# ivargr/kmer_mapper

Measured on AMD Instinct MI355X. Metric: M k-mers mapped/sec (whole node), k=31 150bp reads, higher is better.
Workload: dtype u64

## Files before the change

kmer_mapper_amd/csrc/kmm_radix.hpp:

```cpp
#pragma once
#include <type_traits>
#include "kmm_radix_plan.hpp"

constexpr int RX_NT = 512;
constexpr int RX_KPT = RX_B / RX_NT;
#ifndef RX_LPR2V
#define RX_LPR2V 16
#endif
constexpr int RX_LPR = RX_LPR2V;
constexpr int RX_NG = RX_NT / RX_LPR;
#ifndef RX_RB1
#define RX_RB1 4
#endif
#ifndef RX_RB2
#define RX_RB2 8
#endif
constexpr int RX_SUBCAP = 1024;
#ifndef RX_SUBCAP3V
#define RX_SUBCAP3V 3072
#endif
constexpr int RX_SUBCAP3 = RX_SUBCAP3V;
#ifndef RX_LPR3
#define RX_LPR3 16
#endif
// ... 775 lines not shown
    uint32_t jmax = n_items;
#pragma unroll
    for (int d = 32; d > 0; d >>= 1) {
        const uint32_t o = __shfl_xor(jmax, d);
        jmax = o > jmax ? o : jmax;
    }
    __syncthreads();
    if ((threadIdx.x & 63) == 0)
        s_wave8[threadIdx.x >> 6] = jmax;
    __syncthreads();
    if (c < F1) {
        rx.item_base[c] = ib;
        rx.work_base[c] = wb;
    }
    if (c == 0) {
        uint32_t m = s_wave8[0];
        for (int x = 1; x < 8; ++x)
            m = s_wave8[x] > m ? s_wave8[x] : m;
        rx.item_base[F1] = tot_items;
        rx.work_base[F1] = tot_rows;
        rx.ctrl[0] = tot_items;
        rx.ctrl[1] = tot_rows;
        rx.ctrl[2] = m;
    }
}

template <bool WITH_P>
__global__ void __launch_bounds__(256) k_rx_colscan(RxView rx)
{
    constexpr int RB = 32;
    constexpr int TB = WITH_P ? 32 : 64, CW = 256;
    static_assert(RX_CH % TB == 0 && TB % RB == 0, "a chunk is whole tiles, a tile whole register rounds");
    __shared__ uint32_t tP[WITH_P ? CW : 1][TB + 1];
    __shared__ uint16_t tS[CW][TB + 2];
    const uint32_t F1 = rx.F1, NB = rx.NB;
    const uint32_t b0 = blockIdx.x * RX_CH;
    const uint32_t b1 = b0 + RX_CH < NB ? b0 + RX_CH : NB;
    const size_t ld = F1 + 1;
    const uint32_t lane = threadIdx.x & 63, wave = threadIdx.x >> 6;
    {
    const uint32_t cb = blockIdx.y * CW;
    const uint32_t c = cb + threadIdx.x;
    const uint32_t nc = F1 - cb < (uint32_t)CW ? F1 - cb : (uint32_t)CW;
    uint32_t run = c < F1 ? rx.csum[(size_t)blockIdx.x * F1 + c] : 0u;
    const uint32_t ib = c < F1 ? rx.item_base[c] : 0u;
    for (uint32_t t0 = b0; t0 < b1; t0 += TB) {
        const uint32_t nb = b1 - t0 < (uint32_t)TB ? b1 - t0 : (uint32_t)TB;
        if (c < F1) {
#pragma unroll 1
            for (uint32_t r0 = 0; r0 < (uint32_t)TB; r0 += RB) {
                const uint16_t *p = rx.start1 + (size_t)(t0 + r0) * ld + c;
                uint32_t lo[RB], hi[RB];
#pragma unroll
                for (int u = 0; u < RB; ++u) {
                    lo[u] = r0 + (uint32_t)u < nb ? p[u * ld] : 0u;
                    hi[u] = r0 + (uint32_t)u < nb ? p[u * ld + 1] : 0u;
                }
#pragma unroll
                for (int u = 0; u < RB; ++u) {
                    const uint32_t cnt = hi[u] - lo[u];
                    if constexpr (WITH_P)
                        tP[threadIdx.x][r0 + u] = run;
                    tS[threadIdx.x][r0 + u] = (uint16_t)lo[u];
                    if (cnt) {
                        uint32_t m = (run + RX_B - 1) / RX_B;
                        while ((uint64_t)m * RX_B < (uint64_t)run + cnt) {
                            rx.item_desc[ib + m] = make_uint2(t0 + r0 + u, WITH_P ? c : run);
                            ++m;
                        }
                    }
                    run += cnt;
                }
            }
        }
        __syncthreads();
        if constexpr (WITH_P) {
            const uint32_t bi = lane & 31;
            for (uint32_t cc = wave * 2 + (lane >> 5); cc < nc; cc += 8) {
                if (bi < nb) {
                    rx.P1T[(size_t)(cb + cc) * (NB + 1) + t0 + bi] = tP[cc][bi];
                    rx.S1T[(size_t)(cb + cc) * NB + t0 + bi] = tS[cc][bi];
                }
            }
        } else {
            for (uint32_t cc = wave; cc < nc; cc += 4) {
                if (lane < nb)
                    rx.S1T[(size_t)(cb + cc) * NB + t0 + lane] = tS[cc][lane];
            }
        }
        __syncthreads();
    }
    }
}

constexpr int RX_TR2 = 32;
__global__ void __launch_bounds__(256) k_rx_tr2(RxView rx)
{
    __shared__ uint16_t tile[RX_TR2][RX_MAXF + 2];
    const uint32_t n_items = rx.ctrl[0], cols = rx.F2 + 1;
    const uint32_t i0 = blockIdx.x * RX_TR2;
    if (i0 >= n_items)
        return;
    const uint32_t ni = n_items - i0 < (uint32_t)RX_TR2 ? n_items - i0 : (uint32_t)RX_TR2;
    for (uint32_t e = threadIdx.x; e < ni * cols; e += 256)
        tile[e / cols][e % cols] = rx.start2[(size_t)i0 * cols + e];
    __syncthreads();
    const uint32_t it = threadIdx.x % RX_TR2, c0 = threadIdx.x / RX_TR2;
    if (it < ni)
        for (uint32_t col = c0; col < cols; col += 256 / RX_TR2)
            rx.start2T[(size_t)col * rx.max_items + i0 + it] = tile[it][col];
}

__global__ void __launch_bounds__(RX_NT, 4) k_rx_p2(IndexView iv, RxView rx)
{
    __shared__ uint64_t sbuf[RX_B];
    __shared__ uint32_t sub_src[RX_SUBCAP];
    __shared__ uint32_t sub_meta[RX_SUBCAP], s_wave8[2][RX_NT / 64];
    __shared__ __attribute__((aligned(8))) uint32_t s_cnt[RX_MAXF + 2 + 64];
    __shared__ uint32_t s_base[RX_MAXF + 1], s_wave[4];
    __shared__ uint32_t s_idx;
    const int tid = threadIdx.x, grp = tid / RX_LPR, lg = tid % RX_LPR;
    const uint32_t NB = rx.NB;
    uint32_t gathered = 0;
    uint32_t scan_flip = 0;
    const uint32_t spare = rx_spare_key();
    const int F2 = (int)rx.F2;
    const uint32_t cs = (rx.F1 + 7u) / 8u, limit = rx.ctrl[2] * cs;
    const uint32_t home = rx_xcc_id();
    if (tid <= F2)
        s_cnt[tid] = 0;
    if (tid == 0)
        s_cnt[RX_NT] = 0;
    struct Item {
        uint32_t valid, c, item, b0, lo, hi;
    };
    struct RunDesc {
        uint32_t vs, ve, st;
    };
    auto describe = [&](uint32_t sub, uint32_t idx) {
        Item d;
        d.valid = 0; d.c = 0; d.item = 0; d.b0 = 0; d.lo = 0; d.hi = 0;
        if (idx >= limit)
            return d;
        const uint32_t cj = idx / cs, cc = sub * cs + idx % cs;
        if (cc >= rx.F1)
            return d;
        const uint32_t ib = rx.item_base[cc];
        if (cj >= rx.item_base[cc + 1] - ib)
            return d;
        d.valid = 1;
        d.c = cc;
        d.item = ib + cj;
        d.b0 = rx.item_desc[d.item].x;
        d.lo = cj * RX_B;
        const uint32_t Tc = rx.T1[cc];
        d.hi = Tc - d.lo < (uint32_t)RX_B ? Tc : d.lo + RX_B;
        return d;
    };
    auto run_desc = [&](const Item &d, uint32_t bb) {
        RunDesc r;
        r.vs = 0xFFFFFFFFu; r.ve = 0xFFFFFFFFu; r.st = 0;
        const uint32_t b = bb + tid;
        if (d.valid && b < NB) {
            const uint32_t *P = rx.P1T + (size_t)d.c * (NB + 1);
            r.vs = P[b];
            r.ve = P[b + 1];
            r.st = rx.S1T[(size_t)d.c * NB + b];
        }
        return r;
    };
    RX_PT_DECL;
    for (uint32_t turn = 0; turn < 8u; ++turn) {
    const uint32_t sub = (home + turn) & 7u;
    uint32_t nxt = limit;
    if (tid == 0)
        nxt = rx_pop(rx.queue, sub, limit);
    if (tid == 0)
        s_idx = nxt;
    __syncthreads();
    uint32_t idx = s_idx;
    __syncthreads();
    if (idx >= limit)
        continue;
    if (tid == 0)
        nxt = rx_pop(rx.queue, sub, limit);
    Item it = describe(sub, idx);
    RunDesc rd = run_desc(it, it.b0);
    for (;;) {
        RX_PT(0);
        const uint32_t lo = it.lo, hi = it.hi, n = hi - lo;
        if (it.valid) {
            for (uint32_t bb = it.b0;; bb += RX_NT) {
                if (bb != it.b0)
                    rd = run_desc(it, bb);
                const uint32_t b = bb + tid;
                const uint32_t vs = rd.vs < hi ? rd.vs : hi;
                const bool live = vs < hi;
                const uint32_t ve = live ? rd.ve : vs;
                const uint32_t st = live ? rd.st : 0u;
                const uint32_t from = vs > lo ? vs : lo, to = ve < hi ? ve : hi;
                const uint32_t len = live && to > from ? to - from : 0u;
                const uint64_t src = (uint64_t)b * RX_B + st + (from - vs);
                uint32_t n_sub;
                const uint32_t last_more = (tid == RX_NT - 1 && live && ve < hi) ? 0x80000000u : 0u;
                const uint32_t pre = rx_scan_threads(rx_n_pieces<RX_LPR, true>(len, src) | last_more, s_wave8, scan_flip, &n_sub);
                const bool more = n_sub >> 31;
                n_sub &= 0x7FFFFFFFu;
                RX_PT(1);
                for (uint32_t win = 0; win < n_sub; win += RX_SUBCAP) {
                    rx_list_subruns<RX_LPR, true>(pre, len, src, from - lo, win, sub_src, sub_meta);
                    const uint32_t nw = n_sub - win < (uint32_t)RX_SUBCAP ? n_sub - win : (uint32_t)RX_SUBCAP;
                    rx_pad_list<RX_NG * RX_U2>(nw, sub_src, sub_meta);
                    __syncthreads();
                    for (uint32_t j0 = grp; j0 < nw; j0 += RX_NG * RX_U2) {
                        uint64_t x[RX_U2];
                        uint32_t meta[RX_U2], so[RX_U2];
#pragma unroll
                        for (int u = 0; u < RX_U2; ++u) {
                            meta[u] = sub_meta[j0 + u * RX_NG];
                            so[u] = sub_src[j0 + u * RX_NG];
                        }
#pragma unroll
                        for (int u = 0; u < RX_U2; ++u) {
                            const uint32_t rel = (uint32_t)lg - ((meta[u] >> 6) & 63u);
                            x[u] = rel < (meta[u] & 63u) ? RX_LOAD2(rx.buf1 + ((size_t)so[u] + lg)) : 0ull;
                        }
#pragma unroll
                        for (int u = 0; u < RX_U2; ++u) {
                            const uint32_t rel = (uint32_t)lg - ((meta[u] >> 6) & 63u);
                            if (rel < (meta[u] & 63u))
                                sbuf[(meta[u] >> 12) + rel] = x[u];
                        }
                    }
                    if (more || win + RX_SUBCAP < n_sub)
                        __syncthreads();
                }
                if (!more)
                    break;
            }
        }
        if (tid == 0)
            s_idx = nxt;
        __syncthreads();
        const uint32_t idx_n = s_idx;
        if (tid == 0 && idx_n < limit)
            nxt = rx_pop(rx.queue, sub, limit);
        const Item it_n = describe(sub, idx_n);
        RunDesc rd_n;
        rd_n.vs = 0xFFFFFFFFu; rd_n.ve = 0xFFFFFFFFu; rd_n.st = 0;
        if (it.valid) {
            uint64_t q[RX_KPT];
            uint32_t valid = 0;
#pragma unroll
            for (int i = 0; i < RX_KPT; ++i) {
                const uint32_t e = i * RX_NT + tid;
                q[i] = 0;
                if (e < n) {
                    q[i] = sbuf[e];
                    valid |= 1u << i;
                }
            }
            gathered += (uint32_t)__popc(valid);
            RX_PT(5);
            auto fine = [&](int i) {
                return ((valid >> i) & 1u) ? ((uint32_t)(q[i] >> rx.w) & (uint32_t)(F2 - 1)) : spare;
            };
            auto mid = [&]() { rd_n = run_desc(it_n, it_n.b0); };
            rx_sort_emit<RX_RB2, false, false>(q, fine, F2, sbuf, s_cnt, s_base, s_wave, rx.buf2 + (size_t)it.item * RX_B,
                            rx.start2 + (size_t)it.item * (F2 + 1) RX_PT_ARG2, mid);
        } else {
            rd_n = run_desc(it_n, it_n.b0);
            __syncthreads();
        }
        if (idx_n >= limit)
            break;
        idx = idx_n;
        it = it_n;
        rd = rd_n;
    }
    }
#ifndef RX_PT_P1
    RX_PT_END(iv, 10);
#endif
    rx_stat_add(iv, 2, gathered);
}

__device__ __forceinline__ uint32_t rx_fold2(uint32_t x)
{
    x = (x | (x >> 1)) & 0x55555555u;
    x = (x | (x >> 1)) & 0x33333333u;
    x = (x | (x >> 2)) & 0x0F0F0F0Fu;
    x = (x | (x >> 4)) & 0x00FF00FFu;
    return (x | (x >> 8)) & 0x0000FFFFu;
}
__device__ __forceinline__ uint32_t rx_fold4(uint32_t x)
{
    x = (x | (x >> 1) | (x >> 2) | (x >> 3)) & 0x11111111u;
    x = (x | (x >> 3)) & 0x03030303u;
    x = (x | (x >> 6)) & 0x000F000Fu;
    return (x | (x >> 12)) & 0xFFu;
}

constexpr int P2F_NT = 1024;
constexpr int P2F_KPT = RX_B / P2F_NT;

enum { P2F_NONE = 0, P2F_BITMAP = 1, P2F_SLOT = 2 };
template <int FILTER, bool FSMALL>
__global__ void __launch_bounds__(P2F_NT) k_rx_p2f(IndexView iv, RxView rx)
{
    constexpr bool SLOT = FILTER == P2F_SLOT;
    constexpr int CAPMAX = SLOT ? P2F_SLOTS : RX_B;
    __shared__ __attribute__((aligned(16))) uint32_t s_bits[SLOT ? P2F_SLOT_WORDS : (1 << P2F_LOGBITS) / 32];
    __shared__ __attribute__((aligned(16))) uint64_t sbuf[CAPMAX];
    __shared__ uint32_t t_vs[P2F_NT + 64];
    __shared__ uint32_t t_off[P2F_NT];
    __shared__ uint16_t t_aux[RX_B / 64 + 1];
    __shared__ uint32_t t_last;
    __shared__ uint32_t t_sbits[2][RX_B / 32];
    __shared__ uint32_t t_empty[2];
    __shared__ __attribute__((aligned(8))) uint32_t s_cnt2[2][RX_MAXF + 2 + 64];
    __shared__ uint32_t s_base[RX_MAXF + 1], s_wave[4];
    __shared__ uint32_t s_b0[P2F_KMAX], s_v0[P2F_KMAX];
    __shared__ uint32_t s_tot[3][P2F_NT / 64];
    __shared__ uint32_t s_idx;
    const int tid = threadIdx.x, lane = tid & 63;
    const uint32_t wave = (uint32_t)__builtin_amdgcn_readfirstlane(tid >> 6);
    const uint32_t NB = rx.NB;
    const int F2 = (int)rx.F2, w = rx.w;
    const uint32_t bmask = SLOT ? (1u << P2F_LOGBITS) - 1u : (1u << (rx.w + rx.f2)) - 1u;
    const uint32_t gs = (uint32_t)rx.occ_shift;
    constexpr bool nofilt = FILTER == P2F_NONE;
    const uint32_t nwords = nofilt ? 0u : SLOT ? (uint32_t)P2F_SLOT_WORDS
                                               : (((uint32_t)F2 << w) >> gs) / 32u;
    unsigned long long *const multi_stat =
        &iv.stats[(size_t)(blockIdx.x % KMM_STAT_SHARDS) * KMM_STAT_STRIDE + KMM_STAT_RX_MULTI];
    const uint32_t spare = rx_spare_key();
    uint32_t gathered = 0, dropped = 0;
    const uint32_t cs = (rx.F1 + 7u) / 8u;
    const uint32_t P2F_K = rx.p2f_k;
    const uint32_t limit = ((rx.ctrl[2] + P2F_K - 1u) / P2F_K) * cs;
    const uint32_t home = rx_xcc_id();
    if (tid <= F2)
        s_cnt2[0][tid] = s_cnt2[1][tid] = 0;
    RX_PT_DECL;

    struct RunDesc {
        uint32_t a, b;
    };
    for (uint32_t turn = 0; turn < 8u; ++turn) {
    const uint32_t sub = (home + turn) & 7u;
    for (;;) {
        if (tid == 0)
            s_idx = rx_pop(rx.queue, sub, limit);
        __syncthreads();
        const uint32_t idx = s_idx;
        __syncthreads();
        if (idx >= limit)
            break;
        const uint32_t cu = idx / cs, cc = sub * cs + idx % cs;
        if (cc >= rx.F1)
            continue;
        const uint32_t ib = rx.item_base[cc], n_items_c = rx.item_base[cc + 1] - ib;
        if (cu * P2F_K >= n_items_c)
            continue;
        const uint32_t j0 = cu * P2F_K;
        const uint32_t n_it = n_items_c - j0 < P2F_K ? n_items_c - j0 : P2F_K;
        const uint32_t Tc = rx.T1[cc];
        const uint16_t *S = rx.S1T + (size_t)cc * NB;
        const bool last_c = cc + 1u >= rx.F1;
        const uint16_t *SN = last_c ? rx.start1 + rx.F1 : S + NB;
        const uint32_t sn = last_c ? rx.F1 + 1u : 1u;
        if ((uint32_t)tid < n_it) {
            const uint2 d = rx.item_desc[ib + j0 + tid];
            s_b0[tid] = d.x;
            s_v0[tid] = d.y;
        }
        if (nofilt) {
        } else if (SLOT || gs == 0) {
            const uint4 *src = reinterpret_cast<const uint4 *>((SLOT ? rx.slots : rx.occ) + (size_t)cc * nwords);
            uint4 *dst = reinterpret_cast<uint4 *>(s_bits);
            for (uint32_t i = tid; i < nwords / 4u; i += P2F_NT)
                dst[i] = src[i];
            for (uint32_t i = (nwords & ~3u) + tid; !SLOT && i < nwords; i += P2F_NT)
                s_bits[i] = rx.occ[(size_t)cc * nwords + i];
        } else {
            const uint32_t *src = rx.occ + (((size_t)cc * nwords) << gs);
            for (uint32_t i = tid; i < nwords; i += P2F_NT) {
                uint32_t o = 0;
                if (gs == 1) {
                    const uint2 v = *reinterpret_cast<const uint2 *>(src + 2 * (size_t)i);
                    o = rx_fold2(v.x) | (rx_fold2(v.y) << 16);
                } else {
                    const uint4 v = *reinterpret_cast<const uint4 *>(src + 4 * (size_t)i);
                    o = rx_fold4(v.x) | (rx_fold4(v.y) << 8) | (rx_fold4(v.z) << 16) | (rx_fold4(v.w) << 24);
                }
                s_bits[i] = o;
            }
        }
        if (tid < 2 * (RX_B / 32))
            (&t_sbits[0][0])[tid] = 0u;
        if (tid < 2)
            t_empty[tid] = 0u;
        __syncthreads();

        auto item_lo = [&](uint32_t j) { return (j0 + j) * (uint32_t)RX_B; };
        auto item_n = [&](uint32_t j) {
            const uint32_t lo = (j0 + j) * (uint32_t)RX_B;
            return Tc - lo < (uint32_t)RX_B ? Tc - lo : (uint32_t)RX_B;
        };
        auto load_desc = [&](uint32_t bb) {
            RunDesc r;
            const uint32_t b = bb + tid;
            r.a = 0; r.b = 0;
            if (b < NB) {
                r.a = S[b];
                r.b = SN[b * sn];
            }
            return r;
        };
        auto prescan = [&](RunDesc &r, uint32_t row) {
            const uint32_t len = r.b - r.a;
            r.a |= len << 16;
            r.b = wave_scan_incl(len);
            if (lane == 63)
                s_tot[row][wave] = r.b;
        };
        auto put_table = [&](const RunDesc &r, uint32_t v0, uint32_t row, uint32_t lo, uint32_t hi, int mb = -1) {
            const uint32_t len = r.a >> 16, st = r.a & 0xFFFFu;
            const uint32_t tot = s_tot[row][lane & 15];
            const uint32_t below = (uint32_t)__builtin_amdgcn_readlane((int)wave_scan_incl((uint32_t)lane < wave ? tot : 0u), 15);
            const uint32_t vs = v0 + below + r.b - len, ve = vs + len;
            if (mb >= 0 && vs > lo && vs < hi) {
                if (len > 0u)
                    atomicOr(&t_sbits[mb][(vs - lo) >> 5], 1u << ((vs - lo) & 31u));
                else
                    t_empty[mb] = 1u;
            }
            t_vs[tid] = vs;
            t_off[tid] = (uint32_t)tid * RX_B + st - vs;
            if (tid == P2F_NT - 1) {
                t_vs[P2F_NT] = ve;
                if (ve < hi)
                    t_last = P2F_NT - 1;
            }
            const uint32_t from = vs > lo ? vs : lo, to = ve < hi ? ve : hi;
            if (from < to) {
                for (uint32_t a = (from - lo + 63u) >> 6; lo + (a << 6) < to; ++a)
                    t_aux[a] = (uint16_t)tid;
                if (to == hi)
                    t_last = (uint32_t)tid;
            }
        };
        auto fill = [&](auto merge_tag, uint32_t bb, uint32_t lo, uint32_t n, uint32_t c_lo, uint32_t c_hi,
                        uint64_t (&x)[P2F_KPT], int mb = -1) {
            constexpr bool MERGE = decltype(merge_tag)::value;
            const uint32_t c_end = lo + n < c_hi ? lo + n : c_hi;
            const uint32_t a0 = wave * 8u;
            uint32_t av = 0;
            {
                const uint32_t pa = lo + ((a0 + (uint32_t)lane) << 6);
                const uint32_t ia = a0 + ((uint32_t)lane <= 8u ? (uint32_t)lane : 8u);
                const uint32_t aux = t_aux[ia];
                av = pa < c_lo ? 0u : (pa < c_end ? aux : t_last);
            }
            uint32_t A[P2F_KPT + 1];
#pragma unroll
            for (int i = 0; i <= P2F_KPT; ++i)
                A[i] = (uint32_t)__builtin_amdgcn_readlane((int)av, i);
            uint32_t v[P2F_KPT], pos[P2F_KPT], len_max = 0;
            const uint32_t e0 = (a0 << 6) + (uint32_t)lane;
            auto n_below = [&](uint32_t bound) {
                const int32_t c = ((int32_t)(bound - lo) - (int32_t)e0 + 63) >> 6;
                return (uint32_t)(c < 0 ? 0 : (c > P2F_KPT ? P2F_KPT : c));
            };
            const uint32_t vmask = ((1u << n_below(c_end)) - 1u) & ~((1u << n_below(c_lo)) - 1u);
#pragma unroll
            for (int u = 0; u < P2F_KPT; ++u) {
                v[u] = lo + e0 + ((uint32_t)u << 6);
                pos[u] = A[u];
                const uint32_t len = A[u + 1] > A[u] ? A[u + 1] - A[u] : 0u;
                len_max = len > len_max ? len : len_max;
            }
            bool by_bits = false;
            if (!MERGE && mb >= 0 && t_empty[mb] == 0u) {
                by_bits = true;
                const uint32_t mw = t_sbits[mb][a0 * 2u + ((uint32_t)lane & 15u)];
#pragma unroll
                for (int u = 0; u < P2F_KPT; ++u) {
                    const uint32_t mlo = (uint32_t)__builtin_amdgcn_readlane((int)mw, 2 * u);
                    const uint32_t mhi = (uint32_t)__builtin_amdgcn_readlane((int)mw, 2 * u + 1);
                    const uint64_t m1 = (((uint64_t)mhi << 32) | mlo) >> 1;
                    pos[u] += __builtin_amdgcn_mbcnt_hi((uint32_t)(m1 >> 32), __builtin_amdgcn_mbcnt_lo((uint32_t)m1, 0u));
                }
                len_max = 0;
            }
            if (!by_bits) {
            const uint32_t span = A[P2F_KPT] > A[0] ? A[P2F_KPT] - A[0] : 0u;
            if (span < 64u) {
                const uint32_t sv = t_vs[A[0] + (uint32_t)lane];
#pragma unroll
                for (int u = 0; u < P2F_KPT; ++u) {
                    for (uint32_t i = A[u] + 1u; i <= A[u + 1]; ++i) {
                        const uint32_t st = (uint32_t)__builtin_amdgcn_readlane((int)sv, (int)(i - A[0]));
                        pos[u] += v[u] >= st ? 1u : 0u;
                    }
                }
                len_max = 0;
            }
            }
            for (uint32_t stp = len_max ? 1u << (31 - __builtin_clz(len_max)) : 0u; stp >= 1u; stp >>= 1) {
#pragma unroll
                for (int u = 0; u < P2F_KPT; ++u) {
                    const uint32_t cand = pos[u] + stp;
                    const uint32_t t = t_vs[cand <= A[u + 1] ? cand : A[u + 1]];
                    pos[u] = (cand <= A[u + 1] && t <= v[u]) ? cand : pos[u];
                }
            }
            const uint32_t bbs = (uint32_t)__builtin_amdgcn_readfirstlane((int)bb);
            const char *base = reinterpret_cast<const char *>(rx.buf1 + (size_t)bbs * RX_B);
            const size_t left = (size_t)NB * RX_B - (size_t)bbs * RX_B;
            const uint32_t lim = left > 0x1FFFFFFFull ? 0x1FFFFFFFu : (uint32_t)left - 1u;
#pragma unroll
            for (int u = 0; u < P2F_KPT; ++u) {
                uint32_t el = t_off[pos[u]] + v[u];
                el = el < lim ? el : lim;
                const uint64_t y = RX_LOAD2(reinterpret_cast<const uint64_t *>(base + (el << 3)));
                x[u] = (!MERGE || ((vmask >> u) & 1u)) ? y : x[u];
#if RX_PROBE_P2R
                if (u % RX_PROBE_P2R == 0) {
                    const size_t all = (size_t)NB * RX_B, far = ((size_t)bbs * RX_B + el + all / 2) % all;
                    const uint64_t z = RX_LOAD2(rx.buf1 + far);
                    asm volatile("" ::"v"(z));
                }
#endif
            }
            return vmask;
        };

        uint32_t cover = 0, b0 = 0;
        RunDesc rd;
        rd.a = 0; rd.b = 0;
        auto more_rounds = [&](uint32_t j, uint64_t (&x)[P2F_KPT], uint32_t &vm) {
            const uint32_t lo = item_lo(j), n = item_n(j), hi = lo + n;
            uint32_t bb = b0 + P2F_NT;
            while (cover < hi && bb < NB) {
                RunDesc r2 = load_desc(bb);
                prescan(r2, 2u);
                __syncthreads();
                put_table(r2, cover, 2u, lo, hi);
                __syncthreads();
                const uint32_t cover2 = t_vs[P2F_NT];
                vm |= fill(std::true_type(), bb, lo, n, cover, cover2, x);
                cover = cover2;
                bb += P2F_NT;
            }
            __syncthreads();
        };
        auto process = [&](uint32_t j, uint64_t (&xa)[P2F_KPT], uint32_t vma, uint64_t (&xb)[P2F_KPT], uint32_t &vmb) {
            const uint32_t item = ib + j0 + j;
            RX_PT(0);
            uint32_t keys[P2F_KPT], n_ok = 0;
            if (nofilt) {
#pragma unroll
                for (int u = 0; u < P2F_KPT; ++u) {
                    const uint32_t ok = (vma >> u) & 1u;
                    n_ok += ok;
                    keys[u] = ok ? __builtin_amdgcn_ubfe((uint32_t)xa[u], (uint32_t)w, (uint32_t)rx.f2) : spare;
                }
            } else {
#pragma unroll
                for (int u = 0; u < P2F_KPT; ++u) {
                    const uint32_t xl = (uint32_t)xa[u];
                    const uint32_t bit = SLOT ? rx_filter_slot(xl & bmask, xa[u] >> P2F_LOGBITS)
                                              : (xl & bmask) >> gs;
                    const uint32_t ok = (s_bits[bit >> 5] >> (bit & 31u)) & (vma >> u) & 1u;
                    n_ok += ok;
                    keys[u] = ok ? __builtin_amdgcn_ubfe(xl, (uint32_t)w, (uint32_t)rx.f2) : spare;
                }
            }
            gathered += (uint32_t)__popc(vma);
            dropped += (uint32_t)__popc(vma) - n_ok;
            RX_PT(5);
            if (j + 2u < n_it)
                prescan(rd, j & 1u);
            if (j + 1u < n_it) {
                const uint32_t lo1 = item_lo(j + 1u), n1 = item_n(j + 1u);
                b0 = s_b0[j + 1u];
                cover = t_vs[P2F_NT];
                vmb = fill(std::false_type(), b0, lo1, n1, lo1, cover, xb, (int)((j + 1u) & 1u));
                if (cover < lo1 + n1)
                    more_rounds(j + 1u, xb, vmb);
            }
            RX_PT(1);
            auto fine = [&](int i) { return keys[i]; };
            auto mid = [&]() {
                if (j + 2u < n_it) {
                    put_table(rd, s_v0[j + 2u], j & 1u, item_lo(j + 2u), item_lo(j + 2u) + item_n(j + 2u), (int)(j & 1u));
                    if (j + 3u < n_it)
                        rd = load_desc(s_b0[j + 3u]);
                }
            };
            rx_sort_emit<P2F_KPT, false, true, P2F_NT, false, decltype(fine), decltype(mid), (FSMALL ? 2 : 1), false, RxNoHook, CAPMAX>(
                xa, fine, F2, sbuf, s_cnt2[j & 1u], s_base, s_wave, rx.buf2 + (size_t)item * RX_B,
                rx.start2 + (size_t)item * (F2 + 1) RX_PT_ARG2, mid, P2F_KPT, -1, RxNoHook(),
                RX_PROBE_P2W ? rx.probe + (size_t)item * RX_B : nullptr, RX_PROBE_P2W, SLOT ? rx.p2f_cap : (uint32_t)RX_B,
                SLOT ? multi_stat : nullptr);
            if (tid < RX_B / 32)
                t_sbits[(j + 1u) & 1u][tid] = 0u;
            if (tid == 0)
                t_empty[(j + 1u) & 1u] = 0u;
        };

        uint64_t x0[P2F_KPT], x1[P2F_KPT];
        uint32_t vm0 = 0, vm1 = 0;
        b0 = s_b0[0];
        rd = load_desc(b0);
        prescan(rd, 0u);
        __syncthreads();
        put_table(rd, s_v0[0], 0u, item_lo(0), item_lo(0) + item_n(0), 0);
        if (n_it > 1u) {
            rd = load_desc(s_b0[1]);
            prescan(rd, 1u);
        }
        __syncthreads();
        cover = t_vs[P2F_NT];
        vm0 = fill(std::false_type(), b0, item_lo(0), item_n(0), item_lo(0), cover, x0, 0);
        __syncthreads();
        if (cover < item_lo(0) + item_n(0))
            more_rounds(0, x0, vm0);
        if (tid < RX_B / 32)
            t_sbits[0][tid] = 0u;
        if (tid == 0)
            t_empty[0] = 0u;
        if (n_it > 1u) {
            put_table(rd, s_v0[1], 1u, item_lo(1), item_lo(1) + item_n(1), 1);
            if (n_it > 2u)
                rd = load_desc(s_b0[2]);
        }
        __syncthreads();
        for (uint32_t j = 0; j < n_it; j += 2u) {
            process(j, x0, vm0, x1, vm1);
            if (j + 1u < n_it)
                process(j + 1u, x1, vm1, x0, vm0);
        }
    }
    }
#ifndef RX_PT_P1
    RX_PT_END(iv, 10);
#endif
    rx_stat_add(iv, 2, gathered);
    rx_stat_add(iv, KMM_STAT_RX_DROPPED, dropped);
}

#ifdef RX_P3_FP_STATS
#define RX_P3_KEY_READ(cond) key_reads += (cond) ? 1u : 0u
#else
#define RX_P3_KEY_READ(cond)
#endif
template <int WMAX, int ECAP, int WPS, typename DirT, int SUBCAP = RX_SUBCAP3, bool P16 = false, bool FP = false>
__global__ void __launch_bounds__(RX_NT, WPS) k_rx_p3(IndexView iv, RxView rx, int max_freq)
{
    static_assert(!P16 || sizeof(DirT) == 2, "the 16-bit directory is copied as it is");
    __shared__ uint32_t sfp[FP ? (ECAP + 8) / 4 : 1];
    __shared__ __attribute__((aligned(4))) DirT sdir[WMAX + 2];
    __shared__ uint64_t skeys[ECAP];
    __shared__ uint32_t scnt[ECAP];
    __shared__ uint32_t sub_list[SUBCAP];
    __shared__ uint32_t s_wb[RX_MAXF + 1], s_wave8[2][RX_NT / 64];
    __shared__ uint32_t s_idx;
    const int tid = threadIdx.x, grp = tid / RX_LPR_P3, lg = tid % RX_LPR_P3;
    const uint32_t n_rows = rx.ctrl[1], F1 = rx.F1, F2 = rx.F2;
    const uint32_t W = 1u << rx.w;
    const uint64_t M = iv.modulo;
    for (uint32_t i = tid; i <= F1; i += RX_NT)
        s_wb[i] = rx.work_base[i];
    const uint32_t gs = (F2 + 7u) / 8u, limit = n_rows * gs;
    unsigned long long *counters = rx.queue + 128;
    const uint32_t home = rx_xcc_id();
    uint32_t hits = 0, probed = 0, scan_flip = 0;
#ifdef RX_P3_FP_STATS
    uint32_t key_reads = 0;
#endif
    const int sh = rx.w + rx.f2;
    __syncthreads();
    struct Slice {
        uint32_t valid, g, e0, ne, it0, n_it, over, tot, fmax;
        uint64_t h0;
    };
    auto describe = [&](uint32_t sub, uint32_t idx) {
        Slice d;
        d.valid = 0; d.g = 0; d.e0 = 0; d.ne = 0; d.it0 = 0; d.n_it = 0; d.h0 = 0; d.over = 0; d.tot = 0; d.fmax = 0xFFFFu;
        if (idx >= limit)
            return d;
        const uint32_t row = idx / gs, g = sub * gs + idx % gs;
        uint32_t c_lo = 0, c_hi = F1;
        while (c_hi - c_lo > 1) {
            const uint32_t mid = (c_lo + c_hi) >> 1;
            if (s_wb[mid] <= row)
                c_lo = mid;
            else
                c_hi = mid;
        }
        const uint32_t c = c_lo;
        const uint32_t f2c = rx.PF - c * F2 < F2 ? rx.PF - c * F2 : F2;
        if (g >= f2c)
            return d;
        const uint32_t chunk = row - s_wb[c];
        d.valid = 1;
        d.g = g;
        d.h0 = (uint64_t)(c * F2 + g) << rx.w;
        uint32_t e1;
        if (P16) {
            d.e0 = rx.slice_e0[c * F2 + g];
            e1 = rx.slice_e0[c * F2 + g + 1u];
            d.fmax = rx.slice_fmax ? (uint32_t)rx.slice_fmax[c * F2 + g] : 0xFFFFu;
        } else {
            d.e0 = rx.pstart[d.h0];
            e1 = rx.pstart[d.h0 + W < M ? d.h0 + W : M];
        }
        d.tot = e1 - d.e0;
        d.ne = e1 - d.e0 < (uint32_t)ECAP ? e1 - d.e0 : (uint32_t)ECAP;
        d.over = e1 - d.e0 > (uint32_t)ECAP ? 1u : 0u;
        d.it0 = rx.item_base[c] + chunk * RX_IC;
        const uint32_t it_end = rx.item_base[c + 1];
        d.n_it = it_end - d.it0 < (uint32_t)RX_IC ? it_end - d.it0 : (uint32_t)RX_IC;
        return d;
    };
    RX_PT_DECL;
    for (uint32_t turn = 0; turn < 8u; ++turn) {
    const uint32_t sub = (home + turn) & 7u;
    uint32_t nxt = limit;
    if (tid == 0)
        nxt = rx_pop(counters, sub, limit);
    if (tid == 0)
        s_idx = nxt;
    __syncthreads();
    const uint32_t idx_first = s_idx;
    __syncthreads();
    if (idx_first >= limit)
        continue;
    if (tid == 0)
        nxt = rx_pop(counters, sub, limit);
    Slice sl = describe(sub, idx_first);
    for (;;) {
        RX_PT(0);
        const uint32_t g = sl.g, e0 = sl.e0, ne = sl.ne, it0 = sl.it0, n_it = sl.n_it;
        const uint64_t h0 = sl.h0;
        uint32_t rf[RX_IC / RX_NT], rt[RX_IC / RX_NT];
#pragma unroll
        for (int j = 0; j < RX_IC / RX_NT; ++j)
            rf[j] = rt[j] = 0;
        if (sl.valid) {
        uint32_t dv[WMAX / RX_NT + 1];
        uint64_t kv[ECAP / RX_NT];
        uint32_t fv[ECAP / RX_NT];
#ifndef RX_P3_FMAX
#define RX_P3_FMAX 1
#endif
        const bool need_f = RX_P3_FMAX == 0 || (int)sl.fmax > max_freq;
        if (P16) {
            const uint32_t *p32 = reinterpret_cast<const uint32_t *>(rx.pstart16 + h0);
#pragma unroll
            for (int j = 0; j < WMAX / 2 / RX_NT; ++j) {
                const uint32_t i = tid + j * RX_NT;
                dv[j] = i < W / 2u ? p32[i] : 0u;
            }
            if (W < 2u)
                dv[0] = tid == 0 ? (uint32_t)rx.pstart16[h0] : 0u;
        } else {
#pragma unroll
            for (int j = 0; j <= WMAX / RX_NT; ++j) {
                const uint32_t i = tid + j * RX_NT;
                dv[j] = i <= W ? rx.pstart[h0 + i < M ? h0 + i : M] : 0u;
            }
        }
#pragma unroll
        for (int j = 0; j < ECAP / RX_NT; ++j) {
            const uint32_t i = tid + j * RX_NT;
            kv[j] = i < ne ? rx.pkeys[(size_t)e0 + i] : 0ull;
            fv[j] = i < ne && need_f ? rx.pfreq[(size_t)e0 + i] : 0u;
        }
        const uint16_t *rfp = rx.start2T + (size_t)g * rx.max_items + it0;
        const uint16_t *rtp = rfp + rx.max_items;
#pragma unroll
        for (int j = 0; j < RX_IC / RX_NT; ++j) {
            const uint32_t i = tid + j * RX_NT;
            rf[j] = i < n_it ? rfp[i] : 0u;
            rt[j] = i < n_it ? rtp[i] : 0u;
        }
        if (P16) {
            uint32_t *sd32 = reinterpret_cast<uint32_t *>(sdir);
#pragma unroll
            for (int j = 0; j < WMAX / 2 / RX_NT; ++j) {
                const uint32_t i = tid + j * RX_NT;
                if (i < W / 2u)
                    sd32[i] = dv[j];
            }
            if (W < 2u && tid == 0)
                sdir[0] = (DirT)dv[0];
            if (tid == 0)
                sdir[W] = (DirT)sl.tot;
        } else {
#pragma unroll
            for (int j = 0; j <= WMAX / RX_NT; ++j) {
                const uint32_t i = tid + j * RX_NT;
                if (i <= W)
                    sdir[i] = (DirT)(dv[j] - e0);
            }
        }
#pragma unroll
        for (int j = 0; j < ECAP / RX_NT; ++j) {
            const uint32_t i = tid + j * RX_NT;
            if (i < ne) {
                skeys[i] = kv[j];
                if constexpr (FP)
                    reinterpret_cast<uint8_t *>(sfp)[i] = (uint8_t)rx_p3_fp(kv[j] >> sh);
                scnt[i] = (int)fv[j] <= max_freq ? 0u : RX_FILTERED;
            }
        }
        }
        RX_PT(1);
        if (tid == 0)
            s_idx = nxt;
        __syncthreads();
        const uint32_t idx_n = s_idx;
        if (tid == 0 && idx_n < limit)
            nxt = rx_pop(counters, sub, limit);
        const Slice sl_n = describe(sub, idx_n);
        auto probe_bucket_hbm = [&](uint64_t q, uint32_t st, uint32_t cn) {
            for (uint32_t j = 0; j < cn; ++j) {
                const size_t e = (size_t)e0 + st + j;
                if (rx.pkeys[e] == q && (int)rx.pfreq[e] <= max_freq) {
                    atomicAdd(&rx.ecnt[e], 1u);
                    ++hits;
                }
            }
        };
        if (sl.valid) {
        {
            constexpr int NR = RX_IC / RX_NT;
            uint32_t len[NR], np[NR], np_sum = 0, src[NR];
#pragma unroll
            for (int j = 0; j < NR; ++j) {
                len[j] = rt[j] - rf[j];
                src[j] = (uint32_t)(tid + j * RX_NT) * (uint32_t)RX_B + rf[j];
                np[j] = (len[j] + (uint32_t)RX_LPR_P3 - 1u) / (uint32_t)RX_LPR_P3;
                np_sum += np[j];
            }
            const char *wbase = reinterpret_cast<const char *>(rx.buf2 + (size_t)__builtin_amdgcn_readfirstlane((int)it0) * RX_B);
            uint32_t n_sub;
            const uint32_t pre = rx_scan_threads(np_sum, s_wave8, scan_flip, &n_sub);
            for (uint32_t win = 0; win < n_sub; win += SUBCAP) {
                uint32_t first = pre;
#pragma unroll
                for (int j = 0; j < NR; ++j) {
                    const uint32_t j0 = first > win ? first : win;
                    const uint32_t j1 = first + np[j] < win + (uint32_t)SUBCAP ? first + np[j] : win + (uint32_t)SUBCAP;
                    for (uint32_t q = j0; q < j1; ++q) {
                        const uint32_t done = (q - first) * (uint32_t)RX_LPR_P3;
                        const uint32_t n = len[j] - done < (uint32_t)RX_LPR_P3 ? len[j] - done : (uint32_t)RX_LPR_P3;
                        sub_list[q - win] = ((src[j] + done) << 5) | n;
                    }
                    first += np[j];
                }
                const uint32_t nw = n_sub - win < (uint32_t)SUBCAP ? n_sub - win : (uint32_t)SUBCAP;
                constexpr uint32_t STEP = RX_NG3 * RX_U;
                static_assert(SUBCAP % STEP == 0, "a padded list must fit the window");
                const uint32_t n_bat = (nw + STEP - 1u) / STEP;
                for (uint32_t i = nw + tid; i < n_bat * STEP; i += RX_NT)
                    sub_list[i] = 0u;
                __syncthreads();
                RX_PT(2);
                auto request = [&](uint32_t j0, uint64_t (&x)[RX_U]) {
                    uint32_t e[RX_U], act = 0;
#pragma unroll
                    for (int u = 0; u < RX_U; ++u)
                        e[u] = sub_list[j0 + u * RX_NG3];
#pragma unroll
                    for (int u = 0; u < RX_U; ++u) {
                        const bool in = (uint32_t)lg < (e[u] & 31u);
                        x[u] = RX_LOAD3(reinterpret_cast<const uint64_t *>(wbase + (((e[u] >> 5) + (in ? (uint32_t)lg : 0u)) << 3)));
                        act |= (in ? 1u : 0u) << u;
#if RX_PROBE_P3R
                        if (u % RX_PROBE_P3R == 0) {
                            const size_t far = ((size_t)it0 * RX_B + (e[u] >> 5) + (uint32_t)lg) % ((size_t)rx.NB * RX_B);
                            const uint64_t z = RX_LOAD3(rx.buf1 + far);
                            asm volatile("" ::"v"(z));
                        }
#endif
                    }
                    return act;
                };
                auto probe = [&](auto over_tag, const uint64_t (&x)[RX_U], uint32_t actm) {
                    constexpr bool OVER = decltype(over_tag)::value;
#pragma unroll
                    for (int g0 = 0; g0 < RX_U; g0 += RX_G3) {
                        uint32_t st[RX_G3], cn[RX_G3];
#pragma unroll
                        for (int i = 0; i < RX_G3; ++i) {
                            const uint32_t hb = (uint32_t)x[g0 + i] & (W - 1u);
                            st[i] = sdir[hb];
                            cn[i] = sdir[hb + 1];
                        }
                        uint32_t mx = 0;
#pragma unroll
                        for (int i = 0; i < RX_G3; ++i) {
                            const bool act = (actm >> (g0 + i)) & 1u;
                            probed += act ? 1u : 0u;
                            cn[i] = act ? cn[i] - st[i] : 0u;
                            if constexpr (OVER) {
                                if (cn[i] && st[i] + cn[i] > ne) {
                                    probe_bucket_hbm(x[g0 + i], st[i], cn[i]);
                                    cn[i] = 0;
                                }
                            }
                            mx = cn[i] > mx ? cn[i] : mx;
                        }
                        if constexpr (FP) {
                            uint32_t f0[RX_G3], f1[RX_G3], fp4[RX_G3], cm[RX_G3], any = 0;
#pragma unroll
                            for (int i = 0; i < RX_G3; ++i) {
                                const uint32_t wi = (OVER && !cn[i] ? 0u : st[i]) >> 2;
                                f0[i] = sfp[wi];
                                f1[i] = sfp[wi + 1u];
                            }
#pragma unroll
                            for (int i = 0; i < RX_G3; ++i) {
                                fp4[i] = rx_p3_fp4(x[g0 + i] >> sh);
                                const uint32_t lo = __builtin_amdgcn_alignbit(f1[i], f0[i], 8u * st[i]);
                                cm[i] = rx_p3_match4(lo, fp4[i], cn[i]);
                                any |= cm[i];
                            }
                            while (any) {
                                uint64_t key[RX_G3];
                                uint32_t e8[RX_G3];
#pragma unroll
                                for (int i = 0; i < RX_G3; ++i) {
                                    e8[i] = cm[i] ? 8u * st[i] + (uint32_t)__builtin_ctz(cm[i]) : 0u;
                                    key[i] = *reinterpret_cast<const uint64_t *>(reinterpret_cast<const char *>(skeys) + e8[i]);
                                    RX_P3_KEY_READ(cm[i] != 0u);
// ... 332 lines not shown
```

kmer_mapper_amd/csrc/kmm_radix_plan.hpp:

```cpp
#pragma once
#include <cstddef>
#include <cstdint>
#include <optional>

constexpr int RX_B = 8192;
constexpr int RX_MAXF = 512;
#ifndef RX_CHV
#define RX_CHV 256
#endif
constexpr int RX_CH = RX_CHV;
constexpr int RX_IC = 1024;
constexpr int RX_ECAP = 4096;
constexpr int RX_ECAP_BIG = 8192;
constexpr int RX_ECAP_MID = 4608;
constexpr int P2F_KMAX = 64;
constexpr int P2F_LOGBITS = 19;
constexpr int P2F_SLOT_WORDS = 3 << (P2F_LOGBITS - 6);
constexpr int P2F_SLOTS = 5888;

constexpr uint32_t rx_filter_slot(uint32_t b, uint64_t quot)
{
    const uint32_t v = ((uint32_t)quot ^ (uint32_t)(quot >> 24) ^ (uint32_t)(quot >> 48)) + (b << 23);
    const uint32_t h16 = ((v & 0xFFFFFFu) * 0x9E3779u) >> 16;
    return 3u * (b >> 1) + ((h16 * 3u) >> 16);
}

#if defined(__HIPCC__)
#define RX_PLAN_HD __host__ __device__
#else
#define RX_PLAN_HD
#endif
constexpr int RX_P3_FP_ENTRIES = 5;

RX_PLAN_HD inline uint32_t rx_p3_fp4(uint64_t quot)
{
    const uint32_t v = (uint32_t)quot ^ (uint32_t)(quot >> 24) ^ (uint32_t)(quot >> 48);
#if defined(__HIP_DEVICE_COMPILE__)
    const uint32_t h = __umul24(v, 0xB5297Bu);
    return __builtin_amdgcn_perm(h, h, 0x02020202u);
#else
    return (((v & 0xFFFFFFu) * 0xB5297Bu >> 16) & 0xFFu) * 0x01010101u;
#endif
}
RX_PLAN_HD inline uint32_t rx_p3_fp(uint64_t quot) { return rx_p3_fp4(quot) & 0xFFu; }

RX_PLAN_HD inline uint32_t rx_p3_match4(uint32_t lo, uint32_t fp4, uint32_t cn)
{
    const uint32_t x = lo ^ fp4;
    const uint32_t z = ((x - 0x01010101u) & ~x & 0x80808080u) >> 7;
    const uint32_t width = 8u * cn < 31u ? 8u * cn : 31u;
    return z & ((1u << width) - 1u);
}
RX_PLAN_HD inline uint32_t rx_p3_match_entry4(uint32_t hi, uint32_t fp4, uint32_t cn)
{
    const uint32_t x = hi ^ fp4;
    return cn >= (uint32_t)RX_P3_FP_ENTRIES ? ((x - 1u) & ~x & 0x80u) << 24 : 0u;
}
RX_PLAN_HD inline uint32_t rx_p3_first_entry(uint32_t m) { return ((uint32_t)__builtin_ctz(m) + 1u) >> 3; }

RX_PLAN_HD inline uint32_t rx_p3_candidates(uint64_t f, uint32_t fp, uint32_t cn)
{
    const uint32_t fp4 = fp * 0x01010101u;
    uint32_t m = rx_p3_match4((uint32_t)f, fp4, cn) | rx_p3_match_entry4((uint32_t)(f >> 32), fp4, cn), out = 0;
    for (; m; m &= m - 1u)
        out |= 1u << rx_p3_first_entry(m);
    return out;
}

struct RxGeometry {
    int w = 12, f2 = 0;
    int occ_shift = 0;
    bool slot_filter = false;
    uint32_t PF = 1, F1 = 1, F2 = 1;
};

inline std::optional<RxGeometry> rx_geometry(uint64_t modulo, uint64_t S, bool filter, int w, int maxf = RX_MAXF, int f2_force = -1)
{
    if (w < 0 || w > 13 || modulo == 0 || modulo >= (1ull << 31))
        return std::nullopt;
    const uint64_t PF = (modulo + (1ull << w) - 1) >> w;
    if (PF > (uint64_t)maxf * maxf)
        return std::nullopt;
    int lg = 0;
    while ((1ull << lg) < PF)
        ++lg;
    int f2 = (lg + 1) / 2;
    bool for_filter = false;
    if (filter && w + f2 > P2F_LOGBITS) {
        const double load = S ? (double)S / (double)modulo : 0.5;
        for (int gs = 0; gs <= 2 && !for_filter; ++gs) {
            const int fb = P2F_LOGBITS + gs - w;
            if (fb < 0 || load * (double)(1 << gs) > 0.75)
                continue;
            if (((PF + (1ull << fb) - 1) >> fb) <= (uint64_t)RX_MAXF && fb <= 9) {
                f2 = fb;
                for_filter = true;
            }
        }
    }
    if (f2_force >= 0)
        f2 = f2_force;
    const uint64_t max_quo = ~0ull / modulo;
    auto fits = [&](int sh) { return sh == 0 || (sh < 64 && (max_quo >> (64 - sh)) == 0); };
    while (f2 > 0 && !fits(w + f2))
        --f2;
    if (!fits(w + f2))
        return std::nullopt;
    const uint64_t F2 = 1ull << f2, F1 = (PF + F2 - 1) / F2;
    if (F2 > (uint64_t)maxf || F1 > (uint64_t)(for_filter ? RX_MAXF : maxf))
        return std::nullopt;
    RxGeometry g;
    g.w = w;
    g.f2 = f2;
    g.occ_shift = w + f2 > P2F_LOGBITS ? w + f2 - P2F_LOGBITS : 0;
    g.slot_filter = w + f2 == P2F_LOGBITS;
    g.PF = (uint32_t)PF;
    g.F1 = (uint32_t)F1;
    g.F2 = (uint32_t)F2;
    return g;
}

inline std::optional<RxGeometry> rx_choose_geometry(uint64_t modulo, uint64_t S, bool filter, std::optional<int> w_force = std::nullopt,
                                                    int f2_force = -1)
{
    const bool w_forced = w_force.has_value();
    const double load = (double)S / (double)modulo;
    int w = 12;
    if (w_forced)
        w = *w_force;
    else
        while (w > 0 && (load * (double)(1u << w) * 1.3 + 64.0 > (double)RX_ECAP || (1ull << w) > modulo))
            --w;
    const bool fits13_small = load * 8192.0 * 1.3 + 64.0 <= (double)RX_ECAP;
    const bool fits13 = load * 8192.0 * 1.3 + 64.0 <= (double)RX_ECAP_BIG;
    auto conf = [&](int w_, int maxf) { return rx_geometry(modulo, S, filter, w_, maxf); };
    std::optional<RxGeometry> g = rx_geometry(modulo, S, filter, w, f2_force >= 0 ? RX_MAXF : 256, f2_force);
    if (!g && w == 12 && !w_forced) {
        if (fits13_small)
            g = conf(13, 256);
        if (!g)
            g = conf(12, RX_MAXF);
        if (!g && fits13 && !(g = conf(13, 256)))
            g = conf(13, RX_MAXF);
    } else if (!g) {
        g = conf(w, RX_MAXF);
    }
    return g;
}

struct RxScratch {
    uint32_t chunks;
    size_t max_items;
    size_t start1, P1T, S1T, csum, T1, item_base, work_base, item_desc, start2, start2T, ctrl, queue;
    size_t meta_bytes;
    size_t buf1_bytes, buf2_bytes;
};

constexpr size_t rx_align256(size_t x) { return (x + 255) & ~(size_t)255; }

inline RxScratch rx_scratch(uint32_t NB, uint32_t F1, uint32_t F2)
{
    RxScratch s;
    s.chunks = (NB + RX_CH - 1) / RX_CH;
    s.max_items = (size_t)NB + F1 + 1;
    size_t off = 0;
    auto carve = [&](size_t bytes) { const size_t o = off; off += rx_align256(bytes); return o; };
    s.start1 = carve((size_t)NB * (F1 + 1) * 2);
    s.P1T = carve((size_t)F1 * ((size_t)NB + 1) * 4);
    s.S1T = carve((size_t)F1 * NB * 2);
    s.csum = carve((size_t)s.chunks * F1 * 4);
    s.T1 = carve((size_t)F1 * 4);
    s.item_base = carve((size_t)(F1 + 1) * 4);
    s.work_base = carve((size_t)(F1 + 1) * 4);
    s.item_desc = carve(s.max_items * 8);
    s.start2 = carve(s.max_items * (F2 + 1) * 2);
    s.start2T = carve(s.max_items * (F2 + 1) * 2 + 256);
    s.ctrl = carve(64);
    s.queue = carve(2048);
    s.meta_bytes = off;
    s.buf1_bytes = (size_t)NB * RX_B * 8;
    s.buf2_bytes = s.max_items * RX_B * 8;
    return s;
}

constexpr int64_t RX_SUB_CAP_MAX = ((int64_t)1 << 32) - 2 * RX_B;
constexpr int64_t RX_SUB_CAP_FLOOR = (int64_t)1 << 28;
constexpr int RX_SUB_CAP_AGE = 16;

struct RxSplit {
    int64_t n_sub, max_src;
};

inline RxSplit rx_split(int64_t n_src_total, uint32_t X, int64_t cap)
{
    const int64_t cap_src = (cap / RX_B) / X > 0 ? (cap / RX_B) / X : 1;
    RxSplit s;
    s.n_sub = (n_src_total + cap_src - 1) / cap_src;
    s.max_src = s.n_sub ? (n_src_total + s.n_sub - 1) / s.n_sub : cap_src;
    return s;
}

inline int64_t rx_next_smaller_cap(int64_t n_src_total, uint32_t X, int64_t n_sub)
{
    const int64_t next_src = (n_src_total + n_sub) / (n_sub + 1);
    const int64_t cap = next_src * RX_B * X;
    return cap < RX_SUB_CAP_FLOOR ? RX_SUB_CAP_FLOOR : cap;
}

enum class RxP3Variant {
    W12_DIR16,
    W12,
    W13_SMALL_DIR16,
    W13_SMALL,
    W13_MID_DIR16,
    W13_MID,
    W13_BIG,
};
struct RxP3Shape {
    int keys_in_lds;
    int wg_per_cu;
    bool dir16;
    bool fingerprints = false;
};
constexpr RxP3Shape RX_P3_SHAPES[] = {
    {RX_ECAP, 2, true, true}, {RX_ECAP, 2, false},
    {RX_ECAP, 2, true}, {RX_ECAP, 2, false},
    {RX_ECAP_MID, 2, true}, {RX_ECAP_MID, 2, false},
    {RX_ECAP_BIG, 1, false},
};
constexpr const RxP3Shape &rx_p3_shape(RxP3Variant v) { return RX_P3_SHAPES[(int)v]; }
constexpr int rx_p3_fp_shapes()
{
    int n = 0;
    for (const RxP3Shape &s : RX_P3_SHAPES)
        n += s.fingerprints ? 1 : 0;
    return n;
}

inline RxP3Variant rx_choose_p3(int w, bool fits_small, bool fits_mid, bool p16, uint32_t max_slice, bool no_mid)
{
    if (w <= 12)
        return p16 ? RxP3Variant::W12_DIR16 : RxP3Variant::W12;
    const bool lds16 = p16 || max_slice <= 65535u;
    if (fits_small && lds16)
        return p16 ? RxP3Variant::W13_SMALL_DIR16 : RxP3Variant::W13_SMALL;
    if (fits_mid && lds16 && !no_mid)
        return p16 ? RxP3Variant::W13_MID_DIR16 : RxP3Variant::W13_MID;
    return RxP3Variant::W13_BIG;
}

struct RxViewBytes {
    enum : size_t { pstart = 4, pkeys = 8, pkeys_raw = 8, pfreq = 2, pnodes = 4, porig = 4, ecnt = 4, norder = 4, nnode = 4 };
};
constexpr size_t rx_view_bytes(uint64_t modulo, uint64_t S, bool node_order)
{
    return (size_t)(modulo + 1) * RxViewBytes::pstart +
           (size_t)(S ? S : 1) * (RxViewBytes::pkeys + RxViewBytes::pkeys_raw + RxViewBytes::pfreq + RxViewBytes::pnodes +
                                  RxViewBytes::porig + RxViewBytes::ecnt + (node_order ? RxViewBytes::norder + RxViewBytes::nnode : 0));
}

inline int64_t rx_min_units(uint64_t modulo, uint64_t S)
{
    const double bytes = (double)modulo * 4.0 + (double)S * 14.0;
    const double fixed = 50e-6 + bytes / 2.6e12;
    const double per_kmer_radix = 6.5e-12 * (1.0 + bytes / 40e9);
    const double per_kmer_direct = 1.0 / (bytes < 1e9 ? 60e9 : 38e9);
    const int64_t units = (int64_t)(1.25 * fixed / (per_kmer_direct - per_kmer_radix));
    return units < ((int64_t)1 << 22) ? (int64_t)1 << 22 : units;
}
```

Before: 177,600.

## Limit run-table build to waves covering each item's bucket runs

Each item descriptor now also records how many 64-lane waves are needed to cover its bucket-run range, packed into the high bits of the per-item base value. Only those waves load run descriptors, prescan, and write the table. The cross-wave prefix is now accumulated through shared-memory atomics into s_tot rather than a second wave scan over per-wave totals. This is meant to cut redundant global loads and scan work for items that span few runs, at the cost of extra atomics, an extra descriptor load per item, and a 27-bit limit on bucket indices.

```diff
diff --git a/kmer_mapper_amd/csrc/kmm_radix.hpp b/kmer_mapper_amd/csrc/kmm_radix.hpp
--- a/kmer_mapper_amd/csrc/kmm_radix.hpp
+++ b/kmer_mapper_amd/csrc/kmm_radix.hpp
@@ -1101,6 +1101,7 @@
 }
 
 constexpr int P2F_NT = 1024;
+constexpr int P2F_BBITS = 27;
 constexpr int P2F_KPT = RX_B / P2F_NT;
 
 enum { P2F_NONE = 0, P2F_BITMAP = 1, P2F_SLOT = 2 };
@@ -1141,6 +1142,8 @@
     const uint32_t home = rx_xcc_id();
     if (tid <= F2)
         s_cnt2[0][tid] = s_cnt2[1][tid] = 0;
+    if (tid < 3 * (P2F_NT / 64))
+        (&s_tot[0][0])[tid] = 0u;
     RX_PT_DECL;
 
     struct RunDesc {
@@ -1171,7 +1174,8 @@
         const uint32_t sn = last_c ? rx.F1 + 1u : 1u;
         if ((uint32_t)tid < n_it) {
             const uint2 d = rx.item_desc[ib + j0 + tid];
-            s_b0[tid] = d.x;
+            const uint32_t b_end = j0 + tid + 1u < n_items_c ? rx.item_desc[ib + j0 + tid + 1u].x : NB - 1u;
+            s_b0[tid] = d.x | (rx_p2f_table_waves(d.x, b_end, P2F_NT / 64) - 1u) << P2F_BBITS;
             s_v0[tid] = d.y;
         }
         if (nofilt) {
@@ -1207,27 +1211,34 @@
             const uint32_t lo = (j0 + j) * (uint32_t)RX_B;
             return Tc - lo < (uint32_t)RX_B ? Tc - lo : (uint32_t)RX_B;
         };
-        auto load_desc = [&](uint32_t bb) {
-            RunDesc r;
+        auto item_b0 = [&](uint32_t e) { return e & ((1u << P2F_BBITS) - 1u); };
+        auto item_waves = [&](uint32_t e) { return (uint32_t)__builtin_amdgcn_readfirstlane((int)(e >> P2F_BBITS)) + 1u; };
+        auto load_desc = [&](uint32_t bb, uint32_t nw, RunDesc &r) {
+            if (wave >= nw)
+                return;
             const uint32_t b = bb + tid;
             r.a = 0; r.b = 0;
             if (b < NB) {
                 r.a = S[b];
                 r.b = SN[b * sn];
             }
-            return r;
         };
-        auto prescan = [&](RunDesc &r, uint32_t row) {
+        auto prescan = [&](RunDesc &r, uint32_t row, uint32_t nw) {
+            if (wave >= nw)
+                return;
             const uint32_t len = r.b - r.a;
             r.a |= len << 16;
             r.b = wave_scan_incl(len);
-            if (lane == 63)
-                s_tot[row][wave] = r.b;
+            const uint32_t tot = (uint32_t)__builtin_amdgcn_readlane((int)r.b, 63);
+            if ((uint32_t)lane > wave && (uint32_t)lane < nw)
+                atomicAdd(&s_tot[row][lane], tot);
         };
-        auto put_table = [&](const RunDesc &r, uint32_t v0, uint32_t row, uint32_t lo, uint32_t hi, int mb = -1) {
+        auto put_table = [&](const RunDesc &r, uint32_t v0, uint32_t row, uint32_t nw, uint32_t lo, uint32_t hi, int mb = -1) {
+            if (wave >= nw)
+                return;
             const uint32_t len = r.a >> 16, st = r.a & 0xFFFFu;
-            const uint32_t tot = s_tot[row][lane & 15];
-            const uint32_t below = (uint32_t)__builtin_amdgcn_readlane((int)wave_scan_incl((uint32_t)lane < wave ? tot : 0u), 15);
+            const uint32_t below = s_tot[row][wave];
+            s_tot[row][wave] = 0u;
             const uint32_t vs = v0 + below + r.b - len, ve = vs + len;
             if (mb >= 0 && vs > lo && vs < hi) {
                 if (len > 0u)
@@ -1237,10 +1248,10 @@
             }
             t_vs[tid] = vs;
             t_off[tid] = (uint32_t)tid * RX_B + st - vs;
-            if (tid == P2F_NT - 1) {
+            if ((uint32_t)tid == nw * 64u - 1u) {
                 t_vs[P2F_NT] = ve;
                 if (ve < hi)
-                    t_last = P2F_NT - 1;
+                    t_last = (uint32_t)tid;
             }
             const uint32_t from = vs > lo ? vs : lo, to = ve < hi ? ve : hi;
             if (from < to) {
@@ -1339,14 +1350,23 @@
         uint32_t cover = 0, b0 = 0;
         RunDesc rd;
         rd.a = 0; rd.b = 0;
+        uint32_t rd_nw = 0;
+        auto request_table = [&](uint32_t j) {
+            const uint32_t e = s_b0[j];
+            rd_nw = item_waves(e);
+            load_desc(item_b0(e), rd_nw, rd);
+        };
         auto more_rounds = [&](uint32_t j, uint64_t (&x)[P2F_KPT], uint32_t &vm) {
             const uint32_t lo = item_lo(j), n = item_n(j), hi = lo + n;
-            uint32_t bb = b0 + P2F_NT;
+            constexpr uint32_t NW = P2F_NT / 64;
+            uint32_t bb = b0 + 64u * item_waves(s_b0[j]);
             while (cover < hi && bb < NB) {
-                RunDesc r2 = load_desc(bb);
-                prescan(r2, 2u);
+                RunDesc r2;
+                r2.a = 0; r2.b = 0;
+                load_desc(bb, NW, r2);
+                prescan(r2, 2u, NW);
                 __syncthreads();
-                put_table(r2, cover, 2u, lo, hi);
+                put_table(r2, cover, 2u, NW, lo, hi);
                 __syncthreads();
                 const uint32_t cover2 = t_vs[P2F_NT];
                 vm |= fill(std::true_type(), bb, lo, n, cover, cover2, x);
@@ -1381,10 +1401,10 @@
             dropped += (uint32_t)__popc(vma) - n_ok;
             RX_PT(5);
             if (j + 2u < n_it)
-                prescan(rd, j & 1u);
+                prescan(rd, j & 1u, rd_nw);
             if (j + 1u < n_it) {
                 const uint32_t lo1 = item_lo(j + 1u), n1 = item_n(j + 1u);
-                b0 = s_b0[j + 1u];
+                b0 = item_b0(s_b0[j + 1u]);
                 cover = t_vs[P2F_NT];
                 vmb = fill(std::false_type(), b0, lo1, n1, lo1, cover, xb, (int)((j + 1u) & 1u));
                 if (cover < lo1 + n1)
@@ -1394,9 +1414,9 @@
             auto fine = [&](int i) { return keys[i]; };
             auto mid = [&]() {
                 if (j + 2u < n_it) {
-                    put_table(rd, s_v0[j + 2u], j & 1u, item_lo(j + 2u), item_lo(j + 2u) + item_n(j + 2u), (int)(j & 1u));
+                    put_table(rd, s_v0[j + 2u], j & 1u, rd_nw, item_lo(j + 2u), item_lo(j + 2u) + item_n(j + 2u), (int)(j & 1u));
                     if (j + 3u < n_it)
-                        rd = load_desc(s_b0[j + 3u]);
+                        request_table(j + 3u);
                 }
             };
             rx_sort_emit<P2F_KPT, false, true, P2F_NT, false, decltype(fine), decltype(mid), (FSMALL ? 2 : 1), false, RxNoHook, CAPMAX>(
@@ -1412,14 +1432,14 @@
 
         uint64_t x0[P2F_KPT], x1[P2F_KPT];
         uint32_t vm0 = 0, vm1 = 0;
-        b0 = s_b0[0];
-        rd = load_desc(b0);
-        prescan(rd, 0u);
+        b0 = item_b0(s_b0[0]);
+        request_table(0);
+        prescan(rd, 0u, rd_nw);
         __syncthreads();
-        put_table(rd, s_v0[0], 0u, item_lo(0), item_lo(0) + item_n(0), 0);
+        put_table(rd, s_v0[0], 0u, rd_nw, item_lo(0), item_lo(0) + item_n(0), 0);
         if (n_it > 1u) {
-            rd = load_desc(s_b0[1]);
-            prescan(rd, 1u);
+            request_table(1);
+            prescan(rd, 1u, rd_nw);
         }
         __syncthreads();
         cover = t_vs[P2F_NT];
@@ -1432,9 +1452,9 @@
         if (tid == 0)
             t_empty[0] = 0u;
         if (n_it > 1u) {
-            put_table(rd, s_v0[1], 1u, item_lo(1), item_lo(1) + item_n(1), 1);
+            put_table(rd, s_v0[1], 1u, rd_nw, item_lo(1), item_lo(1) + item_n(1), 1);
             if (n_it > 2u)
-                rd = load_desc(s_b0[2]);
+                request_table(2);
         }
         __syncthreads();
         for (uint32_t j = 0; j < n_it; j += 2u) {
diff --git a/kmer_mapper_amd/csrc/kmm_radix_plan.hpp b/kmer_mapper_amd/csrc/kmm_radix_plan.hpp
--- a/kmer_mapper_amd/csrc/kmm_radix_plan.hpp
+++ b/kmer_mapper_amd/csrc/kmm_radix_plan.hpp
@@ -65,6 +65,13 @@
     for (; m; m &= m - 1u)
         out |= 1u << rx_p3_first_entry(m);
     return out;
+}
+
+constexpr uint32_t rx_p2f_item_runs(uint32_t b0, uint32_t b_end) { return b_end - b0 + 1u; }
+constexpr uint32_t rx_p2f_table_waves(uint32_t b0, uint32_t b_end, uint32_t waves)
+{
+    const uint32_t nw = (rx_p2f_item_runs(b0, b_end) + 63u) / 64u;
+    return nw < 1u ? 1u : (nw < waves ? nw : waves);
 }
 
 struct RxGeometry {
```

Result: no change. 179,400, median of 6 (+1.0%).
